# alpenlabs/dv-pari

Measured on AMD Instinct MI355X. Metric: R1CS constraints/sec (prove), higher is better.
Workload: dtype u32; 1 GPU; Proof::prove, synthetic dense R1CS, 2^20 constraints (BASELINE config #4); log2_constraints=20, n_wires=1048576, msm_pairs_per_proof=6291456, witness=resident in HBM, entry=dvp_prove_dev (Proof::prove with the witness resident), proofs_in_flight=1

## Files before the change

dv-pari_amd/csrc/capi.cpp:

```cpp
#include "common.h"

#include <atomic>
#include <map>
#include <mutex>
#include <vector>
#include <cstring>
#include <cstdlib>
#include <climits>

namespace dvp {
thread_local int64_t g_last_error_index = -1;
thread_local hipError_t g_last_hip_error = hipSuccess;

bool g_prof_enabled = false;
static unsigned g_prof_mask = ~0u;
static std::mutex g_prof_mu;
static double g_prof_ms[PROF_NSLOTS] = {0};
static uint64_t g_prof_n[PROF_NSLOTS] = {0};
struct Pending { int slot; hipEvent_t e0, e1; uint64_t key; };
struct Shape { double ms = 0; uint64_t n = 0; };
static std::map<uint64_t, Shape> g_prof_round0;
static std::vector<Pending> g_prof_pending;
static const char* kProfNames[PROF_NSLOTS] = {"msm_affine_round0", "msm_total", "extend_total", "prove_total", "msm_affine_rest", "msm_sort", "msm_tail"};

// ... 6 lines not shown
  if (!e0) return;
  (void)hipEventRecord(e1, st);
  std::lock_guard<std::mutex> g(g_prof_mu);
  g_prof_pending.push_back({slot, e0, e1, key});
  e0 = e1 = nullptr;
}
void prof_collect() {
  std::lock_guard<std::mutex> g(g_prof_mu);
  for (auto& p : g_prof_pending) {
    float ms = 0;
    if (hipEventSynchronize(p.e1) == hipSuccess && hipEventElapsedTime(&ms, p.e0, p.e1) == hipSuccess) {
      g_prof_ms[p.slot] += ms;
      g_prof_n[p.slot] += (p.slot == PROF_MSM_AFFINE_REST && p.key) ? p.key : 1;
      if (p.slot == PROF_MSM_ACCUM_AFFINE && p.key) { Shape& sh = g_prof_round0[p.key]; sh.ms += ms; sh.n += 1; }
    }
    (void)hipEventDestroy(p.e0);
    (void)hipEventDestroy(p.e1);
  }
  g_prof_pending.clear();
}

static std::atomic<uint64_t> g_host_waits[2];
void count_host_wait(int kind) { g_host_waits[kind & 1].fetch_add(1, std::memory_order_relaxed); }

static void tune_from_env(Tune& t) {
  t = Tune();
  auto geti = [](const char* name, long long dflt) { const char* e = getenv(name); return e ? atoll(e) : dflt; };
  t.msm_c = geti("DVP_MSM_C", t.msm_c);
  t.msm_k = geti("DVP_MSM_K", t.msm_k);
  t.msm_fixed_c = geti("DVP_MSM_FIXED_C", t.msm_fixed_c);
  t.fx_hi = geti("DVP_FX_HI", t.fx_hi);
  const char* m = getenv("DVP_MSM_MODE");
  t.msm_proj = (m && !strcmp(m, "proj")) ? 1 : 0;
  t.msm_aff_min = geti("DVP_MSM_AFF_MIN", t.msm_aff_min);
  t.msm_hex_max = geti("DVP_MSM_HEX_MAX", t.msm_hex_max);
  t.msm_round_pipeline = geti("DVP_MSM_ROUND_PIPELINE", t.msm_round_pipeline);
  t.msm_sort_fused = geti("DVP_MSM_SORT_FUSED", t.msm_sort_fused);
  t.msm_bucket_pairs_max = geti("DVP_MSM_BUCKET_PAIRS_MAX", t.msm_bucket_pairs_max);
  t.msm_aff_bmax = geti("DVP_MSM_AFF_BMAX", t.msm_aff_bmax);
  t.msm_aff_bmin = geti("DVP_MSM_AFF_BMIN", t.msm_aff_bmin);
  t.ecfft_radix4 = geti("DVP_ECFFT_RADIX4", t.ecfft_radix4);
  t.ecfft_fold = geti("DVP_ECFFT_FOLD", t.ecfft_fold);
  t.msm_accum_fast = geti("DVP_MSM_ACCUM_FAST", t.msm_accum_fast);
  t.msm_tail_groups = geti("DVP_MSM_TAIL_GROUPS", t.msm_tail_groups);
  t.msm_accum_hex_max = geti("DVP_MSM_ACCUM_HEX_MAX", t.msm_accum_hex_max);
  t.gf_inv_tabs = geti("DVP_GF_INV_TABS", t.gf_inv_tabs);
  t.msm_ws_slots = geti("DVP_MSM_WS_SLOTS", t.msm_ws_slots);
  t.msm_gate_min = geti("DVP_MSM_GATE_MIN", t.msm_gate_min);
  t.msm_aff_tpb = geti("DVP_MSM_AFF_TPB", t.msm_aff_tpb);
  t.cache_replicas = geti("DVP_CACHE_REPLICAS", t.cache_replicas);
  t.msm_quad_max = geti("DVP_MSM_QUAD_MAX", t.msm_quad_max);
  t.msm_accum_quad_max = geti("DVP_MSM_ACCUM_QUAD_MAX", t.msm_accum_quad_max);
  t.msm_fixed_min = geti("DVP_MSM_FIXED_MIN", t.msm_fixed_min);
  t.horner_max_pub = geti("DVP_HORNER_MAX_PUB", t.horner_max_pub);
  t.fr_bi_shape = geti("DVP_FR_BI_SHAPE", t.fr_bi_shape);
  t.msm_aligned_signed = geti("DVP_MSM_ALIGNED_SIGNED", t.msm_aligned_signed);
  t.prove_host_transcript = geti("DVP_PROVE_HOST_TRANSCRIPT", t.prove_host_transcript);
  t.msm_table_refuse = geti("DVP_MSM_TABLE_REFUSE", t.msm_table_refuse);
  if (const char* e = getenv("DVP_TABLE_BUDGET_BYTES")) {
    const unsigned long long v = strtoull(e, nullptr, 10);
    t.table_budget_bytes = v > (unsigned long long)LLONG_MAX ? -1 : (long long)v;
  }
}
static std::mutex g_dev_mu;
static std::vector<int> g_devices;
std::vector<int> mgpu_devices() {
  std::lock_guard<std::mutex> g(g_dev_mu);
  return g_devices;
}
Tune& tune() {
  static Tune t = [] { Tune x; tune_from_env(x); return x; }();
  return t;
}
}

static long long* tune_slot(const char* name) {
  dvp::Tune& t = dvp::tune();
  struct { const char* n; long long* v; } tab[] = {
      {"DVP_MSM_C", &t.msm_c}, {"DVP_MSM_K", &t.msm_k}, {"DVP_MSM_FIXED_C", &t.msm_fixed_c}, {"DVP_FX_HI", &t.fx_hi},
      {"DVP_MSM_PROJ", &t.msm_proj}, {"DVP_MSM_AFF_MIN", &t.msm_aff_min}, {"DVP_MSM_HEX_MAX", &t.msm_hex_max}, {"DVP_MSM_ROUND_PIPELINE", &t.msm_round_pipeline}, {"DVP_MSM_SORT_FUSED", &t.msm_sort_fused}, {"DVP_MSM_BUCKET_PAIRS_MAX", &t.msm_bucket_pairs_max}, {"DVP_MSM_AFF_BMAX", &t.msm_aff_bmax}, {"DVP_MSM_AFF_BMIN", &t.msm_aff_bmin}, {"DVP_ECFFT_RADIX4", &t.ecfft_radix4}, {"DVP_ECFFT_FOLD", &t.ecfft_fold}, {"DVP_MSM_ACCUM_FAST", &t.msm_accum_fast}, {"DVP_MSM_TAIL_GROUPS", &t.msm_tail_groups}, {"DVP_MSM_ACCUM_HEX_MAX", &t.msm_accum_hex_max}, {"DVP_GF_INV_TABS", &t.gf_inv_tabs}, {"DVP_MSM_WS_SLOTS", &t.msm_ws_slots}, {"DVP_MSM_GATE_MIN", &t.msm_gate_min}, {"DVP_MSM_AFF_TPB", &t.msm_aff_tpb}, {"DVP_CACHE_REPLICAS", &t.cache_replicas},
      {"DVP_MSM_QUAD_MAX", &t.msm_quad_max}, {"DVP_MSM_ACCUM_QUAD_MAX", &t.msm_accum_quad_max}, {"DVP_MSM_FIXED_MIN", &t.msm_fixed_min}, {"DVP_HORNER_MAX_PUB", &t.horner_max_pub}, {"DVP_FR_BI_SHAPE", &t.fr_bi_shape},
      {"DVP_MSM_ALIGNED_SIGNED", &t.msm_aligned_signed}, {"DVP_PROVE_HOST_TRANSCRIPT", &t.prove_host_transcript},
      {"DVP_TABLE_BUDGET_BYTES", &t.table_budget_bytes}, {"DVP_MSM_TABLE_REFUSE", &t.msm_table_refuse}};
  for (auto& e : tab)
    if (!strcmp(name, e.n)) return e.v;
  return nullptr;
}
extern "C" int dvp_tune_set(const char* name, long long value) {
  long long* v = name ? tune_slot(name) : nullptr;
  if (!v) return DVP_EINVAL;
  *v = value;
  return DVP_OK;
}
extern "C" int dvp_tune_get(const char* name, long long* value) {
  long long* v = name ? tune_slot(name) : nullptr;
  if (!v || !value) return DVP_EINVAL;
  *value = *v;
  return DVP_OK;
}
extern "C" void dvp_tune_reset(void) { dvp::tune_from_env(dvp::tune()); }

extern "C" void dvp_profile_enable(int on) {
  dvp::g_prof_mask = on == 2 ? (1u << dvp::PROF_MSM_ACCUM_AFFINE) : ~0u;
  dvp::g_prof_enabled = on != 0;
}
extern "C" void dvp_profile_reset(void) {
  dvp::prof_collect();
  std::lock_guard<std::mutex> g(dvp::g_prof_mu);
  for (int i = 0; i < dvp::PROF_NSLOTS; ++i) { dvp::g_prof_ms[i] = 0; dvp::g_prof_n[i] = 0; }
  dvp::g_prof_round0.clear();
  dvp::g_host_waits[0] = 0;
  dvp::g_host_waits[1] = 0;
}
extern "C" int dvp_profile_round0_shapes(uint64_t* pairs, double* total_ms, uint64_t* launches, int cap) {
  if (cap < 0 || (cap > 0 && (!pairs || !total_ms || !launches))) return DVP_EINVAL;
  dvp::prof_collect();
  std::lock_guard<std::mutex> g(dvp::g_prof_mu);
  int k = 0;
  for (auto& e : dvp::g_prof_round0) {
    if (k < cap) { pairs[k] = e.first; total_ms[k] = e.second.ms; launches[k] = e.second.n; }
    ++k;
  }
  return k;
}
extern "C" int dvp_profile_read(const char* name, double* total_ms, uint64_t* launches) {
  if (!name || !total_ms || !launches) return DVP_EINVAL;
  if (!strcmp(name, "host_waits_stream") || !strcmp(name, "host_waits_side")) {
    *total_ms = 0;
    *launches = dvp::g_host_waits[name[11] == 's' && name[12] == 'i' ? 1 : 0].load();
    return DVP_OK;
  }
  dvp::prof_collect();
  std::lock_guard<std::mutex> g(dvp::g_prof_mu);
  for (int i = 0; i < dvp::PROF_NSLOTS; ++i)
    if (!strcmp(name, dvp::kProfNames[i])) { *total_ms = dvp::g_prof_ms[i]; *launches = dvp::g_prof_n[i]; return DVP_OK; }
  return DVP_EINVAL;
}

extern "C" const char* dvp_strerror(int s) {
  switch (s) {
    case DVP_OK: return "ok";
    case DVP_EINVAL: return "invalid argument (size, null pointer or non-canonical field element)";
    case DVP_EDECODE: return "invalid xsk233 point encoding";
    case DVP_EUNSAT: return "R1CS constraint not satisfied by the witness";
    case DVP_EHIP: return "HIP runtime error";
    case DVP_EIO: return "I/O error";
    case DVP_ENOMEM: return "out of memory";
    case DVP_ECHALLENGE: return "Fiat-Shamir challenge lies in the evaluation domain";
    default: return "unknown status";
  }
}

// ... 27 lines not shown
```

dv-pari_amd/csrc/common.h:

```cpp
#pragma once
#include <hip/hip_runtime.h>
#include <stdint.h>
#include <stdio.h>

#include <vector>

#include "../../include/dvpari_internal.h"

namespace dvp {

extern thread_local int64_t g_last_error_index;
extern thread_local hipError_t g_last_hip_error;

inline int hip_fail(hipError_t e, const char* what, const char* file, int line) {
  g_last_hip_error = e;
  fprintf(stderr, "[dvpari] HIP error %d (%s) at %s:%d: %s\n", (int)e, hipGetErrorString(e), file, line, what);
  if (e == hipErrorOutOfMemory) {
    (void)hipGetLastError();
    return DVP_ENOMEM;
  }
  return DVP_EHIP;
}

#define DVP_HIP(call)                                                        \
// ... 40 lines not shown
struct Tune {
  long long msm_c = 0;
  long long msm_k = 0;
  long long msm_fixed_c = 0;
  long long fx_hi = -1;
  long long msm_proj = 0;
  long long msm_aff_min = 1ll << 19;
  long long msm_gate_min = 1;
  long long msm_ws_slots = 2;
  long long cache_replicas = 1;
  long long msm_aff_tpb = 256;
  long long msm_aff_bmin = 8;
  long long msm_aff_bmax = 136;
  long long ecfft_radix4 = 3;
  long long ecfft_fold = 1;
  long long msm_accum_fast = 1;
  long long msm_tail_groups = 1;
  long long msm_accum_hex_max = -1;
  long long gf_inv_tabs = 1;
  long long msm_accum_quad_max = 0;
  long long msm_bucket_pairs_max = 12;
  long long msm_sort_fused = 1;
  long long msm_round_pipeline = 2;
  long long msm_hex_max = -1;
  long long msm_quad_max = 0;
  long long msm_fixed_min = 1ll << 16;
  long long fr_bi_shape = 6;
  long long horner_max_pub = -1;
  long long prove_host_transcript = 0;
  long long table_budget_bytes = -1;
  long long msm_table_refuse = 0;
  long long msm_aligned_signed = 1;
};
Tune& tune();

std::vector<int> mgpu_devices();

inline unsigned cdiv(size_t a, size_t b) { return (unsigned)((a + b - 1) / b); }

enum ProfSlot { PROF_MSM_ACCUM_AFFINE = 0, PROF_MSM_TOTAL, PROF_EXTEND_TOTAL, PROF_PROVE_TOTAL, PROF_MSM_AFFINE_REST, PROF_MSM_SORT, PROF_MSM_TAIL, PROF_NSLOTS };
extern bool g_prof_enabled;
struct ProfScope {
  int slot;
  hipStream_t st;
  hipEvent_t e0 = nullptr, e1 = nullptr;
  uint64_t key = 0;
  ProfScope(int slot_, hipStream_t st_, uint64_t key_ = 0);
  void stop();
};
void prof_collect();
void count_host_wait(int kind);

}
```

dv-pari_amd/csrc/msm.hip:

```cpp
#include <algorithm>
#include <cstdlib>
#include <cstring>
#include <atomic>
#include <chrono>
#include <mutex>
#include <type_traits>
#include <vector>

#include "common.h"
#include "k233.cuh"
#include "tau.cuh"
#include "codec.cuh"

namespace dvp {

constexpr uint32_t FXW_VALID = 0x80000000u, FXW_KEY_MASK = 0xfffffu, FXW_NEG = 0x10000000u, ITEM_NEG = 0x80000000u;
constexpr int FXW_ROW_SHIFT = 20;
__host__ __device__ __forceinline__ uint32_t fxw_key(uint32_t d) { return d & FXW_KEY_MASK; }
__host__ __device__ __forceinline__ uint32_t fxw_row(uint32_t d) { return (d >> FXW_ROW_SHIFT) & 0xffu; }

template <class DIGIT>
__global__ void __launch_bounds__(256)
k_recode(const uint32_t* __restrict__ scalars, const uint8_t* __restrict__ inf, uint32_t n, int c, int W, int n_narrow,
         DIGIT* __restrict__ digits, unsigned long long* __restrict__ err) {
// ... 1030 lines not shown
  const uint32_t base = blockIdx.x * SCAN_BLK + threadIdx.x * SCAN_EPT;
  for (int r = 1; r <= R; ++r) {
    uint32_t* o = rp + (size_t)(2 * (r - 1) + 1) * ((size_t)m + 1);
    const uint32_t add = bs[(size_t)(r - 1) * gridDim.x + blockIdx.x];
    if (r == 1 && off0) {
#pragma unroll
      for (int k = 0; k < SCAN_EPT; ++k)
        if (base + k < m) {
          const uint32_t v = o[base + k] + add, c = cnt0[base + k];
          o[base + k] = v;
          off0[base + k] = 2u * v;
          if (c & 1u) items[2u * v + c] = AFF_NONE;
        }
      continue;
    }
#pragma unroll
    for (int k = 0; k < SCAN_EPT; ++k)
      if (base + k < m) o[base + k] += add;
  }
}
struct DescPlan {
  unsigned long long at[40];
};
template <int LPK>
__global__ void __launch_bounds__(1024)
k_round_desc_all(const uint32_t* __restrict__ rp, uint32_t nkeys, int R, DescPlan plan, uint32_t* __restrict__ desc) {
  const uint32_t gid = blockIdx.x * blockDim.x + threadIdx.x;
  const uint32_t key = gid / LPK, lane = gid % LPK;
  if (key >= nkeys) return;
  const size_t stride = (size_t)nkeys + 1;
  for (int r0 = 1; r0 < R; r0 += 8) {
    uint32_t cr[8], o[8], oo[8];
#pragma unroll
    for (int q = 0; q < 8; ++q) {
      const int r = r0 + q;
      if (r < R) {
        const uint32_t* c = rp + (size_t)(2 * (r - 1)) * stride;
        cr[q] = c[key];
        o[q] = c[stride + key];
        oo[q] = c[3 * stride + key];
      } else {
        cr[q] = 0; o[q] = 0; oo[q] = 0;
      }
    }
#pragma unroll
    for (int q = 0; q < 8; ++q) {
      const int r = r0 + q;
      if (r >= R) break;
      const uint32_t nout = (cr[q] + 1) >> 1;
      uint32_t* d = desc + plan.at[r];
      for (uint32_t j = lane; j < nout; j += LPK) d[oo[q] + j] = (o[q] + 2 * j) | ((2 * j + 1 < cr[q]) ? DESC_PAIR : 0u);
    }
  }
}

template <int LPK>
__global__ void __launch_bounds__(256)
k_round_desc(const uint32_t* __restrict__ cnt, const uint32_t* __restrict__ off, const uint32_t* __restrict__ ooff ,
             uint32_t nkeys, uint32_t* __restrict__ desc) {
  const uint32_t gid = blockIdx.x * blockDim.x + threadIdx.x;
  const uint32_t key = gid / LPK, lane = gid % LPK;
  if (key >= nkeys) return;
  const uint32_t c = cnt[key], o = off[key], oo = ooff[key], nout = (c + 1) >> 1;
  for (uint32_t j = lane; j < nout; j += LPK) desc[oo + j] = (o + 2 * j) | ((2 * j + 1 < c) ? DESC_PAIR : 0u);
}

#ifndef AFF_PRIO
#define AFF_PRIO 1
#endif
#ifndef AFF_XY
#define AFF_XY 1
#endif
__device__ __forceinline__ void aff_set_prio(uint32_t v) {
  switch (v % 3u) {
    case 0: __builtin_amdgcn_s_setprio(0); break;
    case 1: __builtin_amdgcn_s_setprio(1); break;
    default: __builtin_amdgcn_s_setprio(2); break;
  }
}
constexpr uint32_t AFF_BMAX = 136;
__device__ __forceinline__ uint32_t aff_slots_per_thread(uint32_t total, uint32_t cap, uint32_t bmax_bmin) {
  const uint32_t bmax = bmax_bmin & 0xffu, bmin = (bmax_bmin >> 8) & 0xffu;
  const uint32_t units = (total + cap - 1) / cap;
  const uint32_t R = (units + bmax - 1) / bmax;
  const uint32_t B = R ? (units + R - 1) / R : 1;
  return B < bmin ? bmin : B;
}
struct WaveTrace {
  unsigned long long* buf;
  uint32_t cap, tag;
};
template <bool FIRST, bool TRACE = false>
__global__ void __launch_bounds__(EC_TPB) __attribute__((amdgpu_waves_per_eu(3, 3)))
k_affine_round(const Aff* __restrict__ pts, const uint2* __restrict__ desc, const uint32_t* __restrict__ total_ptr ,
               uint32_t cap, uint32_t bmax, GfSqrTables T, Gf* __restrict__ prefix, Aff* __restrict__ out, uint32_t sign_mask, WaveTrace wt) {
  extern __shared__ char lds_raw[];
  unsigned long long tr_t0 = 0, tr_c0 = 0, tr_t1 = 0, tr_t2 = 0;
  if (TRACE) { tr_t0 = wall_clock64(); tr_c0 = clock64(); }
  GfLdsK L = gf_ldsk_init(lds_raw);
#if AFF_PRIO
  const uint32_t wslot = __builtin_amdgcn_s_getreg(((4 - 1) << 11) | 4);
#endif
  const uint32_t sm = FIRST ? sign_mask : 0u;
  auto ldx = [&](uint32_t v) -> Gf { return pts[v & ~sm].x; };
  auto ldy = [&](uint32_t v, const Gf& x) -> Gf {
    Gf y = pts[v & ~sm].y;
    if (v & sm) y = gf_add(y, x);
    return y;
  };
  const uint32_t total = *total_ptr;
  const int B = (int)aff_slots_per_thread(total, cap, bmax);
  const uint32_t nthr = (total + B - 1) / B;
  const uint32_t tid = blockIdx.x * blockDim.x + threadIdx.x;
  if (tid >= nthr) return;
  const uint2 none = make_uint2(AFF_NONE, AFF_NONE);
  auto ld_desc = [&](int k) -> uint2 {
    const uint32_t sk = (uint32_t)k * nthr + tid;
    const bool ok = k >= 0 && k < B && sk < total;
    if (FIRST) {
      uint2 v = none;
      if (ok) v = desc[sk];
      return v;
    }
    const uint32_t d = ((const uint32_t*)desc)[ok ? sk : 0u], a = d & ~DESC_PAIR;
    return make_uint2(ok ? a : AFF_NONE, (ok && (d & DESC_PAIR)) ? a + 1 : AFF_NONE);
  };
  const Gf one = gf_one();
  Gf run = one;
  {
    uint2 d0 = ld_desc(0), d1 = ld_desc(1);
    Gf xa = gf_zero(), xb = gf_zero();
    if (d0.y != AFF_NONE) { xa = ldx(d0.x); xb = ldx(d0.y); }
#pragma unroll 1
    for (int k = 0; k < B; ++k) {
#if AFF_PRIO
      aff_set_prio(wslot + (uint32_t)k);
#endif
      const uint2 d2 = ld_desc(k + 2);
      Gf nxa = gf_zero(), nxb = gf_zero();
      if (d1.y != AFF_NONE) { nxa = ldx(d1.x); nxb = ldx(d1.y); }
      Gf den = one;
      if (d0.y != AFF_NONE && !gf_is_zero(xa) && !gf_is_zero(xb)) {
        Gf dd = gf_add(xa, xb);
        if (!gf_is_zero(dd)) den = dd;
        else if (gf_eq(ldy(d0.x, xa), ldy(d0.y, xb))) den = xa;
      }
      prefix[(size_t)k * nthr + tid] = run;
      run = gf_mul(run, den, L);
      d0 = d1; d1 = d2; xa = nxa; xb = nxb;
    }
  }
  if (TRACE) tr_t1 = wall_clock64();
  Gf inv = gf_inv_fast(run, T, L);
  if (TRACE) tr_t2 = wall_clock64();
  {
    uint2 e0 = ld_desc(B - 1), e1 = ld_desc(B - 2);
    Gf px = gf_zero(), qx = gf_zero(), pre = one;
    if (e0.x != AFF_NONE) px = ldx(e0.x);
    if (e0.y != AFF_NONE) { qx = ldx(e0.y); pre = prefix[(size_t)(B - 1) * nthr + tid]; }
#if AFF_XY
    Gf py = gf_zero(), qy = gf_zero();
    if (e0.x != AFF_NONE) py = ldy(e0.x, px);
    if (e0.y != AFF_NONE) qy = ldy(e0.y, qx);
#endif
#pragma unroll 1
    for (int k = B - 1; k >= 0; --k) {
#if AFF_PRIO
      aff_set_prio(wslot + (uint32_t)k);
#endif
      const uint2 e2 = ld_desc(k - 2);
#if AFF_XY
      Gf npx = gf_zero(), nqx = gf_zero(), npy = gf_zero(), nqy = gf_zero(), npre = one;
      if (e1.x != AFF_NONE) { npx = ldx(e1.x); npy = ldy(e1.x, npx); }
      if (e1.y != AFF_NONE) { nqx = ldx(e1.y); nqy = ldy(e1.y, nqx); npre = prefix[(size_t)(k - 1) * nthr + tid]; }
#else
      Gf py = gf_zero(), qy = gf_zero();
      if (e0.x != AFF_NONE) py = ldy(e0.x, px);
      if (e0.y != AFF_NONE) qy = ldy(e0.y, qx);
      Gf npx = gf_zero(), nqx = gf_zero(), npre = one;
      if (e1.x != AFF_NONE) npx = ldx(e1.x);
      if (e1.y != AFF_NONE) { nqx = ldx(e1.y); npre = prefix[(size_t)(k - 1) * nthr + tid]; }
#endif
      if (e0.x != AFF_NONE) {
        const uint32_t sidx = (uint32_t)k * nthr + tid;
        Gf ox = px, oy = py;
        if (e0.y != AFF_NONE) {
          if (gf_is_zero(px)) { ox = qx; oy = qy; }
          else if (!gf_is_zero(qx)) {
            Gf dd = gf_add(px, qx);
            const bool same_x = gf_is_zero(dd);
            const bool dbl = same_x && gf_eq(py, qy);
            if (same_x && !dbl) {
              ox = gf_zero(); oy = gf_zero();
            } else {
              Gf den = dbl ? px : dd;
              Gf dinv, inv_next;
              gf_mul2(pre, den, inv, L, dinv, inv_next);
              inv = inv_next;
              Gf num = dbl ? py : gf_add(py, qy);
              Gf lam = gf_mul(num, dinv, L);
              if (dbl) lam = gf_add(lam, px);
              ox = gf_add(gf_add(gf_sqr(lam), lam), dd);
              oy = gf_add(gf_add(gf_mul(gf_add(px, ox), lam, L), ox), py);
            }
          }
        }
        out[sidx].x = ox; out[sidx].y = oy;
      }
      e0 = e1; e1 = e2; px = npx; qx = nqx; pre = npre;
#if AFF_XY
      py = npy; qy = nqy;
#endif
    }
  }
#if AFF_PRIO
  __builtin_amdgcn_s_setprio(0);
#endif
  if (TRACE) {
    const unsigned long long t3 = wall_clock64(), c3 = clock64();
    if ((threadIdx.x & 63u) == 0) {
      const unsigned long long i = atomicAdd(wt.buf, 1ull);
      if (i < wt.cap) {
        unsigned long long* r = wt.buf + 8 + 8 * i;
        r[0] = tr_t0; r[1] = tr_t1; r[2] = tr_t2; r[3] = t3;
        r[4] = tr_c0; r[5] = c3;
        r[6] = (unsigned long long)__builtin_amdgcn_s_getreg((31 << 11) | 4) | ((unsigned long long)__builtin_amdgcn_s_getreg((31 << 11) | 20) << 32);
        r[7] = (unsigned long long)blockIdx.x | ((unsigned long long)wt.tag << 32) | ((unsigned long long)(uint32_t)B << 48);
      }
    }
  }
}

__global__ void __launch_bounds__(256)
k_bucket_gather_aff(const Aff* __restrict__ in, const uint32_t* __restrict__ cnt, const uint32_t* __restrict__ off,
// ... 497 lines not shown
    static std::mutex attr_mu;
    static bool attr_done[MSM_MAX_DEVICES] = {false};
    std::lock_guard<std::mutex> ga(attr_mu);
    if (!attr_done[cur_dev]) {
      hipError_t attr_err = hipFuncSetAttribute((const void*)k_scatter_local, hipFuncAttributeMaxDynamicSharedMemorySize, 131072);
      if (attr_err == hipSuccess)
        attr_err = hipFuncSetAttribute((const void*)k_hist_local, hipFuncAttributeMaxDynamicSharedMemorySize, 65536);
      if (attr_err == hipSuccess)
        attr_err = hipFuncSetAttribute((const void*)k_scatter_local2, hipFuncAttributeMaxDynamicSharedMemorySize, 131072);
      if (attr_err == hipSuccess)
        attr_err = hipFuncSetAttribute((const void*)k_hist_local2, hipFuncAttributeMaxDynamicSharedMemorySize, 65536);
      if (attr_err == hipSuccess)
        attr_err = hipFuncSetAttribute((const void*)k_part_scatter_staged, hipFuncAttributeMaxDynamicSharedMemorySize, FX_STAGE1_LDS);
      if (attr_err == hipSuccess)
        attr_err = hipFuncSetAttribute((const void*)k_part_scatter_signed<true>, hipFuncAttributeMaxDynamicSharedMemorySize, FX_STAGE1_LDS);
      if (attr_err == hipSuccess)
        attr_err = hipFuncSetAttribute((const void*)k_scatter_local2_staged, hipFuncAttributeMaxDynamicSharedMemorySize, FX_STAGE2_LDS);
      const void* ec[] = {(const void*)k_accum_affine<true, false>, (const void*)k_accum_affine<false, false>, (const void*)k_accum_affine<true, true>,
                          (const void*)k_accum_affine<false, true>, (const void*)k_accum_proj<1>, (const void*)k_accum_proj<4>, (const void*)k_accum_proj<16>,
                          (const void*)k_accum_affine_fast<true, false>, (const void*)k_accum_affine_fast<false, false>, (const void*)k_accum_affine_fast<true, true>,
                          (const void*)k_accum_affine_fast<false, true>, (const void*)k_accum_affine_rest<true>, (const void*)k_accum_affine_rest<false>,
                          (const void*)k_tail_groups, (const void*)k_merge<1, false>, (const void*)k_merge<4, false>, (const void*)k_merge<16, false>, (const void*)k_merge<1, true>, (const void*)k_merge<4, true>, (const void*)k_merge<16, true>,
                          (const void*)k_affine_round<true, false>, (const void*)k_affine_round<false, false>, (const void*)k_affine_round<true, true>,
                          (const void*)k_affine_round<false, true>, (const void*)k_sum_points, (const void*)k_tail<false>, (const void*)k_tail<true>,
                          (const void*)k_bucket_pairs, (const void*)k_bucket_rest};
      for (const void* f : ec)
        if (attr_err == hipSuccess) attr_err = hipFuncSetAttribute(f, hipFuncAttributeMaxDynamicSharedMemorySize, EC_LDS_Q);
      DVP_HIP(attr_err);
      attr_done[cur_dev] = true;
    }
  }
  MsmPlan p = msm_plan(n, fx);
  const FxBits fb = fx ? fx->bits() : FxBits{0, 0};
  const uint32_t FX_NP = fb.np();
  std::unique_lock<std::mutex> g;
  int ws_slot = 0;
  const int ws_slots = tune().msm_ws_slots >= 1 && tune().msm_ws_slots <= MSM_WS_SLOTS ? (int)tune().msm_ws_slots : 1;
  for (int pass = 0; pass < 2 && !g.owns_lock(); ++pass)
    for (int sl = 0; sl < ws_slots && !g.owns_lock(); ++sl) {
      g = std::unique_lock<std::mutex>(g_ws_dev[cur_dev][sl].mu, std::try_to_lock);
      if (g.owns_lock() && pass == 0 && g_ws_dev[cur_dev][sl].busy_for(st)) g.unlock();
      if (g.owns_lock()) ws_slot = sl;
    }
  if (!g.owns_lock()) g = std::unique_lock<std::mutex>(g_ws_dev[cur_dev][0].mu);
  MsmWorkspace& g_ws = g_ws_dev[cur_dev][ws_slot];
  if (g_ws.busy_valid) {
    if (g_ws.busy_stream != st) DVP_HIP(hipStreamWaitEvent(st, g_ws.ev_busy, 0));
// ... 19 lines not shown
  size_t o_ntask = carve(((size_t)p.nkeys + 1) * 4);
  size_t o_toff = carve(((size_t)p.nkeys + 1) * 4);
  size_t o_cnt2 = carve(((size_t)p.nkeys + 1) * 4);
  size_t o_off2 = carve(((size_t)p.nkeys + 1) * 4);
  size_t o_bsum = carve(((size_t)p.nkeys / SCAN_BLK + 8) * 4);
  size_t o_items = carve((p.e_max + (size_t)p.nkeys + 2) * 4);
  const size_t sort_cells = fx ? ((size_t)(fx_nblk + FX_NP + 1) << fb.lo) : ((size_t)p.W * cdiv(n, SORT_CHUNK) << p.c);
  size_t o_hist16 = carve(sort_cells * 2);
  size_t o_choff = carve(sort_cells * 4);
  size_t o_bufA = carve(p.t1_max * sizeof(Ld));
  size_t o_bufB = carve(p.t2_max * sizeof(Ld));
  const Tune tn = tune();
  const bool affine_mode = !tn.msm_proj;
  const size_t affA_n = p.e_max / 2 + p.nkeys + 1, affB_n = p.e_max / 4 + p.nkeys + 1;
  size_t o_affA = carve(affine_mode ? affA_n * sizeof(Aff) : 16);
  size_t o_affB = carve(affine_mode ? affB_n * sizeof(Aff) : 16);
  size_t o_prefix = carve(affine_mode ? (affA_n + 256) * sizeof(Gf) : 16);
  const size_t aff_min = (size_t)(tn.msm_aff_min > 0 ? tn.msm_aff_min : 1);
  const size_t e_est = (size_t)n * (size_t)((fx && fx->signed_digits) ? p.W : (234 + p.c - 1) / p.c);
  int ra_plan = 0;
  while (affine_mode && ra_plan < 40 && (e_est >> (ra_plan + 1)) >= aff_min) ++ra_plan;
  const bool pipelined = affine_mode && tn.msm_round_pipeline != 0 && ra_plan >= 2 && e_est >= 4 * (size_t)p.nkeys;
  const bool side_stream = pipelined && tn.msm_round_pipeline == 1;
  std::vector<size_t> desc_at((size_t)ra_plan + 1, 0);
  size_t desc_n = affA_n + 64;
  if (pipelined) {
    size_t cap_r = p.e_max + p.nkeys, at = 0;
    for (int r = 0; r < ra_plan; ++r) {
      const size_t out_max = cap_r / 2 + p.nkeys + 1;
      if (r >= 1) { desc_at[r] = at; at += out_max + 64; }
      cap_r = out_max;
    }
    if (at > desc_n) desc_n = at;
  }
  size_t o_gdesc = carve(affine_mode ? desc_n * sizeof(uint32_t) : 16);
  size_t o_rp = carve(pipelined ? (size_t)ra_plan * 2 * ((size_t)p.nkeys + 1) * 4 : 16);
  size_t o_bsum2 = carve(((size_t)((ra_plan > 0 ? ra_plan : 1) + 1) * ((size_t)p.nkeys / SCAN_BLK + 1) + 8) * 4);
  size_t o_bkt = carve((size_t)p.nkeys * sizeof(Ld));
  const size_t rest_cap = (size_t)p.nkeys + 2 + p.e_max / (size_t)(p.K > 0 ? p.K : 1);
  size_t o_rest = carve(rest_cap * 4);
  const uint32_t tail_groups = ((uint32_t)(p.W * p.c) + 15u) / 16u;
  size_t o_tail = carve(((size_t)2 * p.W * p.c + 1 + 2 * (size_t)tail_groups) * sizeof(Ld));
  DVP_TRY(g_ws.ensure(o, g_ws_need[cur_dev]));
  char* base = (char*)g_ws.p;
  auto* err = (unsigned long long*)(base + o_err);
  auto* digits = (uint16_t*)(base + o_digits);
  auto* digits32 = (uint32_t*)(base + o_digits32);
  auto* plo = (uint16_t*)(base + o_plo);
  auto* pid = (uint32_t*)(base + o_pid);
  auto* phist = (uint32_t*)(base + o_phist);
  auto* pbase = (uint32_t*)(base + o_pbase);
  auto* ctot = (uint32_t*)(base + o_ctot);
  auto* pstart = (uint32_t*)(base + o_pstart);
// ... 41 lines not shown
    DVP_HIP(hipStreamWaitEvent(g_ws.aux, g_ws.ev, 0));
    DVP_HIP(hipMemcpyAsync(g_ws.pinned, d_max, 4, hipMemcpyDeviceToHost, g_ws.aux));
    return DVP_OK;
  };
  const bool sort_done_by_mscan = pipelined && !side_stream;
  auto prepare_rounds = [&]() -> int {
    if (!pipelined) return DVP_OK;
    hipStream_t bk = st;
    if (side_stream) {
      DVP_TRY(g_ws.ensure_side(1));
      DVP_HIP(hipEventRecord(g_ws.ev_pre, st));
      DVP_HIP(hipStreamWaitEvent(g_ws.side, g_ws.ev_pre, 0));
      bk = g_ws.side;
    }
    const uint32_t nb = cdiv(nk, SCAN_BLK);
    uint32_t* off0 = side_stream ? nullptr : off;
    hipLaunchKernelGGL(k_mscan_local, dim3(nb), dim3(SCAN_TPB), 0, bk, cnt, nk, ra_plan, rp, bsum2);
    hipLaunchKernelGGL(k_mscan_bsums, dim3(ra_plan), dim3(SCAN_TPB), 0, bk, bsum2, nb, nk, rp, off0, off0 ? d_max : (uint32_t*)nullptr);
    if (off0) DVP_TRY(read_max());
    hipLaunchKernelGGL(k_mscan_add, dim3(nb), dim3(SCAN_TPB), 0, bk, rp, bsum2, nk, ra_plan, (const uint32_t*)cnt, off0, items);
    DescPlan plan;
    for (int q = 0; q < 40; ++q) plan.at[q] = q < ra_plan ? desc_at[q] : 0;
    const size_t per_key = (e_est >> 2) / nk;
    if (per_key >= 48)
      hipLaunchKernelGGL((k_round_desc_all<64>), dim3(cdiv((size_t)nk * 64, 1024)), dim3(1024), 0, bk, rp, nk, ra_plan, plan, gdesc);
    else if (per_key >= 8)
      hipLaunchKernelGGL((k_round_desc_all<16>), dim3(cdiv((size_t)nk * 16, 1024)), dim3(1024), 0, bk, rp, nk, ra_plan, plan, gdesc);
    else
      hipLaunchKernelGGL((k_round_desc_all<4>), dim3(cdiv((size_t)nk * 4, 1024)), dim3(1024), 0, bk, rp, nk, ra_plan, plan, gdesc);
    if (side_stream) DVP_HIP(hipEventRecord(g_ws.ev_side[0], g_ws.side));
    DVP_HIP(hipGetLastError());
    prepared = ra_plan;
    return DVP_OK;
  };
  ProfScope ps_total(PROF_MSM_TOTAL, st);
  ProfScope ps_sort(PROF_MSM_SORT, st);
  if (!g_ws.ctrl_clean) {
    DVP_HIP(hipMemsetAsync(err, 0xff, 8, st));
    DVP_HIP(hipMemsetAsync(err + 1, 0, 8, st));
  }
  g_ws.ctrl_clean = false;
  if (fused1)
    ;
  else if (fx && fx->signed_digits)
    hipLaunchKernelGGL(k_recode_signed, dim3(cdiv(n, 256)), dim3(256), 0, st, (const uint32_t*)d_scalars, (const uint8_t*)d_inf, (uint32_t)n,
                       p.c, p.W, p.n_narrow, digits32, err);
  else if (fx)
    hipLaunchKernelGGL((k_recode<uint32_t>), dim3(cdiv(n, 256)), dim3(256), 0, st, (const uint32_t*)d_scalars, (const uint8_t*)d_inf,
                       (uint32_t)n, p.c, p.W, p.n_narrow, digits32, err);
  else
    hipLaunchKernelGGL((k_recode<uint16_t>), dim3(cdiv(n, 256)), dim3(256), 0, st, (const uint32_t*)d_scalars, (const uint8_t*)d_inf,
                       (uint32_t)n, p.c, p.W, p.n_narrow, digits, err);
// ... 59 lines not shown
  const uint32_t aff_lds = (aff_tpb / 64) * GF_LDSK_BYTES_PER_WAVE;
  DVP_HIP(hipOccupancyMaxActiveBlocksPerMultiprocessor(&blk_per_cu, (const void*)k_affine_round<false, false>, (int)aff_tpb, aff_lds));
  if (blk_per_cu < 1) blk_per_cu = 1;
  const uint32_t aff_cap = (uint32_t)n_cu * (uint32_t)blk_per_cu * aff_tpb;
  const uint32_t aff_bmax_only = tn.msm_aff_bmax >= 1 && tn.msm_aff_bmax <= 255 ? (uint32_t)tn.msm_aff_bmax : AFF_BMAX;
  const uint32_t aff_bmin = tn.msm_aff_bmin >= 1 && (uint32_t)tn.msm_aff_bmin <= aff_bmax_only ? (uint32_t)tn.msm_aff_bmin : 1u;
  const uint32_t aff_bmax = aff_bmax_only | (aff_bmin << 8);
  unsigned long long* wt_buf = nullptr;
  uint32_t wt_cap = 0;
  wave_trace_snapshot(&wt_buf, &wt_cap);
  const bool wt_on = wt_buf != nullptr;
  auto launch_round = [&](int r, const uint32_t* d_total, const uint2* dsc) -> int {
    size_t out_max = cap / 2 + nk + 1;
    Aff* outp = (r & 1) ? affB : affA;
    const uint32_t r_max = cdiv(cdiv(out_max, aff_cap), aff_bmax_only);
    const uint32_t grid = r_max * (aff_cap / aff_tpb) + 1;
    {
      ProfScope ps0(r == 0 ? PROF_MSM_ACCUM_AFFINE : -1, st, (uint64_t)n);
      WaveTrace wt{wt_buf, wt_cap, g_wave_trace_tag.fetch_add(wt_on ? 1u : 0u)};
      if (r == 0 && wt.buf)
        hipLaunchKernelGGL((k_affine_round<true, true>), dim3(grid), dim3(aff_tpb), aff_lds, st, pts_in, dsc, d_total, aff_cap, aff_bmax, Tsq, prefix, outp, sign_mask, wt);
      else if (r == 0)
        hipLaunchKernelGGL((k_affine_round<true, false>), dim3(grid), dim3(aff_tpb), aff_lds, st, pts_in, dsc, d_total, aff_cap, aff_bmax, Tsq, prefix, outp, sign_mask, wt);
      else if (wt.buf)
        hipLaunchKernelGGL((k_affine_round<false, true>), dim3(grid), dim3(aff_tpb), aff_lds, st, pts_in, dsc, d_total, aff_cap, aff_bmax, Tsq, prefix, outp, 0u, wt);
      else
        hipLaunchKernelGGL((k_affine_round<false, false>), dim3(grid), dim3(aff_tpb), aff_lds, st, pts_in, dsc, d_total, aff_cap, aff_bmax, Tsq, prefix, outp, 0u, wt);
      ps0.stop();
    }
    pts_in = outp;
    cap = out_max;
    return DVP_OK;
  };
  auto run_round = [&](int r) -> int {
    if (pipelined) {
      if (r == 0 && side_stream) DVP_HIP(hipStreamWaitEvent(st, g_ws.ev_side[0], 0));
      DVP_TRY(launch_round(r, ro(r + 1) + nk, r == 0 ? (const uint2*)items : (const uint2*)(const void*)(gdesc + desc_at[r])));
      return DVP_OK;
    }
    const int nxt = (cur + 1) % 3;
    if (r == 0) {
      if (!(r0_offsets_ready && cur == 0))
        hipLaunchKernelGGL(k_round0_offsets, dim3(cdiv(nk + 1, 256)), dim3(256), 0, st, pc[cur], po[cur], nk, pc[nxt], po[nxt]);
    } else
      DVP_TRY(bookkeep(r, pc[cur], po[cur], pc[nxt], po[nxt], gdesc, st, bsum));
    DVP_TRY(launch_round(r, po[nxt] + nk, r == 0 ? (const uint2*)items : (const uint2*)(const void*)gdesc));
    cur = nxt;
    return DVP_OK;
  };
  int launched = 0;
  std::unique_lock<std::mutex> heavy;
// ... 525 lines not shown
```

Measured before the change: 56.07 million constraints/s.

## Fold numerator into batched-inversion prefix and add optional dense round descriptors

The affine round kernel now multiplies the pair numerator (ya+yb) into the forward prefix product, so the backward pass yields lambda directly from a single paired multiply instead of an inverse followed by a separate multiply. This removes one field multiply and the qy load from the backward pass, at the cost of loading both y coordinates in the forward pass. It also adds an opt-in dense descriptor layout for later rounds that carries explicit output slots and skips wave iterations with no pairs, plus counters for later-round launches. The dense layout doubles descriptor storage and is off by default.

```diff
diff --git a/dv-pari_amd/csrc/capi.cpp b/dv-pari_amd/csrc/capi.cpp
--- a/dv-pari_amd/csrc/capi.cpp
+++ b/dv-pari_amd/csrc/capi.cpp
@@ -52,6 +52,8 @@
 
 static std::atomic<uint64_t> g_host_waits[2];
 void count_host_wait(int kind) { g_host_waits[kind & 1].fetch_add(1, std::memory_order_relaxed); }
+static std::atomic<uint64_t> g_later_rounds[2];
+void count_later_round(bool dense) { g_later_rounds[dense ? 1 : 0].fetch_add(1, std::memory_order_relaxed); }
 
 static void tune_from_env(Tune& t) {
   t = Tune();
@@ -65,6 +67,7 @@
   t.msm_aff_min = geti("DVP_MSM_AFF_MIN", t.msm_aff_min);
   t.msm_hex_max = geti("DVP_MSM_HEX_MAX", t.msm_hex_max);
   t.msm_round_pipeline = geti("DVP_MSM_ROUND_PIPELINE", t.msm_round_pipeline);
+  t.msm_round_dense = geti("DVP_MSM_ROUND_DENSE", t.msm_round_dense);
   t.msm_sort_fused = geti("DVP_MSM_SORT_FUSED", t.msm_sort_fused);
   t.msm_bucket_pairs_max = geti("DVP_MSM_BUCKET_PAIRS_MAX", t.msm_bucket_pairs_max);
   t.msm_aff_bmax = geti("DVP_MSM_AFF_BMAX", t.msm_aff_bmax);
@@ -108,7 +111,7 @@
   dvp::Tune& t = dvp::tune();
   struct { const char* n; long long* v; } tab[] = {
       {"DVP_MSM_C", &t.msm_c}, {"DVP_MSM_K", &t.msm_k}, {"DVP_MSM_FIXED_C", &t.msm_fixed_c}, {"DVP_FX_HI", &t.fx_hi},
-      {"DVP_MSM_PROJ", &t.msm_proj}, {"DVP_MSM_AFF_MIN", &t.msm_aff_min}, {"DVP_MSM_HEX_MAX", &t.msm_hex_max}, {"DVP_MSM_ROUND_PIPELINE", &t.msm_round_pipeline}, {"DVP_MSM_SORT_FUSED", &t.msm_sort_fused}, {"DVP_MSM_BUCKET_PAIRS_MAX", &t.msm_bucket_pairs_max}, {"DVP_MSM_AFF_BMAX", &t.msm_aff_bmax}, {"DVP_MSM_AFF_BMIN", &t.msm_aff_bmin}, {"DVP_ECFFT_RADIX4", &t.ecfft_radix4}, {"DVP_ECFFT_FOLD", &t.ecfft_fold}, {"DVP_MSM_ACCUM_FAST", &t.msm_accum_fast}, {"DVP_MSM_TAIL_GROUPS", &t.msm_tail_groups}, {"DVP_MSM_ACCUM_HEX_MAX", &t.msm_accum_hex_max}, {"DVP_GF_INV_TABS", &t.gf_inv_tabs}, {"DVP_MSM_WS_SLOTS", &t.msm_ws_slots}, {"DVP_MSM_GATE_MIN", &t.msm_gate_min}, {"DVP_MSM_AFF_TPB", &t.msm_aff_tpb}, {"DVP_CACHE_REPLICAS", &t.cache_replicas},
+      {"DVP_MSM_PROJ", &t.msm_proj}, {"DVP_MSM_AFF_MIN", &t.msm_aff_min}, {"DVP_MSM_HEX_MAX", &t.msm_hex_max}, {"DVP_MSM_ROUND_PIPELINE", &t.msm_round_pipeline}, {"DVP_MSM_ROUND_DENSE", &t.msm_round_dense}, {"DVP_MSM_SORT_FUSED", &t.msm_sort_fused}, {"DVP_MSM_BUCKET_PAIRS_MAX", &t.msm_bucket_pairs_max}, {"DVP_MSM_AFF_BMAX", &t.msm_aff_bmax}, {"DVP_MSM_AFF_BMIN", &t.msm_aff_bmin}, {"DVP_ECFFT_RADIX4", &t.ecfft_radix4}, {"DVP_ECFFT_FOLD", &t.ecfft_fold}, {"DVP_MSM_ACCUM_FAST", &t.msm_accum_fast}, {"DVP_MSM_TAIL_GROUPS", &t.msm_tail_groups}, {"DVP_MSM_ACCUM_HEX_MAX", &t.msm_accum_hex_max}, {"DVP_GF_INV_TABS", &t.gf_inv_tabs}, {"DVP_MSM_WS_SLOTS", &t.msm_ws_slots}, {"DVP_MSM_GATE_MIN", &t.msm_gate_min}, {"DVP_MSM_AFF_TPB", &t.msm_aff_tpb}, {"DVP_CACHE_REPLICAS", &t.cache_replicas},
       {"DVP_MSM_QUAD_MAX", &t.msm_quad_max}, {"DVP_MSM_ACCUM_QUAD_MAX", &t.msm_accum_quad_max}, {"DVP_MSM_FIXED_MIN", &t.msm_fixed_min}, {"DVP_HORNER_MAX_PUB", &t.horner_max_pub}, {"DVP_FR_BI_SHAPE", &t.fr_bi_shape},
       {"DVP_MSM_ALIGNED_SIGNED", &t.msm_aligned_signed}, {"DVP_PROVE_HOST_TRANSCRIPT", &t.prove_host_transcript},
       {"DVP_TABLE_BUDGET_BYTES", &t.table_budget_bytes}, {"DVP_MSM_TABLE_REFUSE", &t.msm_table_refuse}};
@@ -141,6 +144,8 @@
   dvp::g_prof_round0.clear();
   dvp::g_host_waits[0] = 0;
   dvp::g_host_waits[1] = 0;
+  dvp::g_later_rounds[0] = 0;
+  dvp::g_later_rounds[1] = 0;
 }
 extern "C" int dvp_profile_round0_shapes(uint64_t* pairs, double* total_ms, uint64_t* launches, int cap) {
   if (cap < 0 || (cap > 0 && (!pairs || !total_ms || !launches))) return DVP_EINVAL;
@@ -158,6 +163,11 @@
   if (!strcmp(name, "host_waits_stream") || !strcmp(name, "host_waits_side")) {
     *total_ms = 0;
     *launches = dvp::g_host_waits[name[11] == 's' && name[12] == 'i' ? 1 : 0].load();
+    return DVP_OK;
+  }
+  if (!strcmp(name, "later_rounds_word") || !strcmp(name, "later_rounds_dense")) {
+    *total_ms = 0;
+    *launches = dvp::g_later_rounds[name[13] == 'd' ? 1 : 0].load();
     return DVP_OK;
   }
   dvp::prof_collect();
diff --git a/dv-pari_amd/csrc/common.h b/dv-pari_amd/csrc/common.h
--- a/dv-pari_amd/csrc/common.h
+++ b/dv-pari_amd/csrc/common.h
@@ -86,6 +86,7 @@
   long long msm_bucket_pairs_max = 12;
   long long msm_sort_fused = 1;
   long long msm_round_pipeline = 2;
+  long long msm_round_dense = 0;
   long long msm_hex_max = -1;
   long long msm_quad_max = 0;
   long long msm_fixed_min = 1ll << 16;
@@ -114,5 +115,6 @@
 };
 void prof_collect();
 void count_host_wait(int kind);
+void count_later_round(bool dense);
 
 }
diff --git a/dv-pari_amd/csrc/msm.hip b/dv-pari_amd/csrc/msm.hip
--- a/dv-pari_amd/csrc/msm.hip
+++ b/dv-pari_amd/csrc/msm.hip
@@ -1076,7 +1076,7 @@
 struct DescPlan {
   unsigned long long at[40];
 };
-template <int LPK>
+template <int LPK, bool DENSE>
 __global__ void __launch_bounds__(1024)
 k_round_desc_all(const uint32_t* __restrict__ rp, uint32_t nkeys, int R, DescPlan plan, uint32_t* __restrict__ desc) {
   const uint32_t gid = blockIdx.x * blockDim.x + threadIdx.x;
@@ -1084,7 +1084,7 @@
   if (key >= nkeys) return;
   const size_t stride = (size_t)nkeys + 1;
   for (int r0 = 1; r0 < R; r0 += 8) {
-    uint32_t cr[8], o[8], oo[8];
+    uint32_t cr[8], o[8], oo[8], A[8];
 #pragma unroll
     for (int q = 0; q < 8; ++q) {
       const int r = r0 + q;
@@ -1093,8 +1093,9 @@
         cr[q] = c[key];
         o[q] = c[stride + key];
         oo[q] = c[3 * stride + key];
+        A[q] = DENSE ? c[stride + nkeys] - c[3 * stride + nkeys] : 0u;
       } else {
-        cr[q] = 0; o[q] = 0; oo[q] = 0;
+        cr[q] = 0; o[q] = 0; oo[q] = 0; A[q] = 0;
       }
     }
 #pragma unroll
@@ -1103,6 +1104,13 @@
       if (r >= R) break;
       const uint32_t nout = (cr[q] + 1) >> 1;
       uint32_t* d = desc + plan.at[r];
+      if (DENSE) {
+        const uint32_t npair = cr[q] >> 1, a = o[q] - oo[q];
+        uint2* d2 = (uint2*)d;
+        for (uint32_t j = lane; j < npair; j += LPK) d2[a + j] = make_uint2((o[q] + 2 * j) | DESC_PAIR, oo[q] + j);
+        if ((cr[q] & 1u) && lane == npair % LPK) d2[A[q] + (2 * oo[q] - o[q])] = make_uint2(o[q] + cr[q] - 1, oo[q] + npair);
+        continue;
+      }
       for (uint32_t j = lane; j < nout; j += LPK) d[oo[q] + j] = (o[q] + 2 * j) | ((2 * j + 1 < cr[q]) ? DESC_PAIR : 0u);
     }
   }
@@ -1125,6 +1133,9 @@
 #ifndef AFF_XY
 #define AFF_XY 1
 #endif
+#ifndef AFF_NUM1
+#define AFF_NUM1 1
+#endif
 __device__ __forceinline__ void aff_set_prio(uint32_t v) {
   switch (v % 3u) {
     case 0: __builtin_amdgcn_s_setprio(0); break;
@@ -1144,7 +1155,10 @@
   unsigned long long* buf;
   uint32_t cap, tag;
 };
-template <bool FIRST, bool TRACE = false>
+struct AffSlot {
+  uint32_t a, b, o;
+};
+template <bool FIRST, bool TRACE = false, bool DENSE = false>
 __global__ void __launch_bounds__(EC_TPB) __attribute__((amdgpu_waves_per_eu(3, 3)))
 k_affine_round(const Aff* __restrict__ pts, const uint2* __restrict__ desc, const uint32_t* __restrict__ total_ptr ,
                uint32_t cap, uint32_t bmax, GfSqrTables T, Gf* __restrict__ prefix, Aff* __restrict__ out, uint32_t sign_mask, WaveTrace wt) {
@@ -1168,91 +1182,141 @@
   const uint32_t tid = blockIdx.x * blockDim.x + threadIdx.x;
   if (tid >= nthr) return;
   const uint2 none = make_uint2(AFF_NONE, AFF_NONE);
-  auto ld_desc = [&](int k) -> uint2 {
+  auto ld_desc = [&](int k) -> AffSlot {
     const uint32_t sk = (uint32_t)k * nthr + tid;
     const bool ok = k >= 0 && k < B && sk < total;
     if (FIRST) {
       uint2 v = none;
       if (ok) v = desc[sk];
-      return v;
-    }
-    const uint32_t d = ((const uint32_t*)desc)[ok ? sk : 0u], a = d & ~DESC_PAIR;
-    return make_uint2(ok ? a : AFF_NONE, (ok && (d & DESC_PAIR)) ? a + 1 : AFF_NONE);
+      return AffSlot{v.x, v.y, 0u};
+    }
+    const uint2 d = DENSE ? desc[ok ? sk : 0u] : make_uint2(((const uint32_t*)desc)[ok ? sk : 0u], 0u);
+    const uint32_t a = d.x & ~DESC_PAIR;
+    return AffSlot{ok ? a : AFF_NONE, (ok && (d.x & DESC_PAIR)) ? a + 1 : AFF_NONE, d.y};
   };
   const Gf one = gf_one();
   Gf run = one;
   {
-    uint2 d0 = ld_desc(0), d1 = ld_desc(1);
+    AffSlot d0 = ld_desc(0), d1 = ld_desc(1);
     Gf xa = gf_zero(), xb = gf_zero();
-    if (d0.y != AFF_NONE) { xa = ldx(d0.x); xb = ldx(d0.y); }
+    if (d0.b != AFF_NONE) { xa = ldx(d0.a); xb = ldx(d0.b); }
+#if AFF_NUM1
+    Gf ya = gf_zero(), yb = gf_zero();
+    if (d0.b != AFF_NONE) { ya = ldy(d0.a, xa); yb = ldy(d0.b, xb); }
+#endif
 #pragma unroll 1
     for (int k = 0; k < B; ++k) {
 #if AFF_PRIO
       aff_set_prio(wslot + (uint32_t)k);
 #endif
-      const uint2 d2 = ld_desc(k + 2);
+      const AffSlot d2 = ld_desc(k + 2);
       Gf nxa = gf_zero(), nxb = gf_zero();
-      if (d1.y != AFF_NONE) { nxa = ldx(d1.x); nxb = ldx(d1.y); }
-      Gf den = one;
-      if (d0.y != AFF_NONE && !gf_is_zero(xa) && !gf_is_zero(xb)) {
-        Gf dd = gf_add(xa, xb);
-        if (!gf_is_zero(dd)) den = dd;
-        else if (gf_eq(ldy(d0.x, xa), ldy(d0.y, xb))) den = xa;
+      if (d1.b != AFF_NONE) { nxa = ldx(d1.a); nxb = ldx(d1.b); }
+#if AFF_NUM1
+      Gf nya = gf_zero(), nyb = gf_zero();
+      if (d1.b != AFF_NONE) { nya = ldy(d1.a, nxa); nyb = ldy(d1.b, nxb); }
+#endif
+      const bool pair = d0.b != AFF_NONE;
+      if (!DENSE || __any(pair)) {
+        Gf den = one;
+#if AFF_NUM1
+        Gf num = gf_zero();
+        if (pair && !gf_is_zero(xa) && !gf_is_zero(xb)) {
+          const Gf dd = gf_add(xa, xb), ys = gf_add(ya, yb);
+          if (!gf_is_zero(dd)) { den = dd; num = ys; }
+          else if (gf_is_zero(ys)) { den = xa; num = ya; }
+        }
+        Gf np, nrun;
+        gf_mul2(num, den, run, L, np, nrun);
+        if (pair) prefix[(size_t)k * nthr + tid] = np;
+        run = nrun;
+#else
+        if (pair && !gf_is_zero(xa) && !gf_is_zero(xb)) {
+          Gf dd = gf_add(xa, xb);
+          if (!gf_is_zero(dd)) den = dd;
+          else if (gf_eq(ldy(d0.a, xa), ldy(d0.b, xb))) den = xa;
+        }
+        if (pair) prefix[(size_t)k * nthr + tid] = run;
+        run = gf_mul(run, den, L);
+#endif
       }
-      prefix[(size_t)k * nthr + tid] = run;
-      run = gf_mul(run, den, L);
       d0 = d1; d1 = d2; xa = nxa; xb = nxb;
+#if AFF_NUM1
+      ya = nya; yb = nyb;
+#endif
     }
   }
   if (TRACE) tr_t1 = wall_clock64();
   Gf inv = gf_inv_fast(run, T, L);
   if (TRACE) tr_t2 = wall_clock64();
   {
-    uint2 e0 = ld_desc(B - 1), e1 = ld_desc(B - 2);
+    AffSlot e0 = ld_desc(B - 1), e1 = ld_desc(B - 2);
     Gf px = gf_zero(), qx = gf_zero(), pre = one;
-    if (e0.x != AFF_NONE) px = ldx(e0.x);
-    if (e0.y != AFF_NONE) { qx = ldx(e0.y); pre = prefix[(size_t)(B - 1) * nthr + tid]; }
+    if (e0.a != AFF_NONE) px = ldx(e0.a);
+    if (e0.b != AFF_NONE) { qx = ldx(e0.b); pre = prefix[(size_t)(B - 1) * nthr + tid]; }
 #if AFF_XY
-    Gf py = gf_zero(), qy = gf_zero();
-    if (e0.x != AFF_NONE) py = ldy(e0.x, px);
-    if (e0.y != AFF_NONE) qy = ldy(e0.y, qx);
+    Gf py = gf_zero();
+    if (e0.a != AFF_NONE) py = ldy(e0.a, px);
+#if !AFF_NUM1
+    Gf qy = gf_zero();
+    if (e0.b != AFF_NONE) qy = ldy(e0.b, qx);
+#endif
 #endif
 #pragma unroll 1
     for (int k = B - 1; k >= 0; --k) {
 #if AFF_PRIO
       aff_set_prio(wslot + (uint32_t)k);
 #endif
-      const uint2 e2 = ld_desc(k - 2);
+      const AffSlot e2 = ld_desc(k - 2);
 #if AFF_XY
-      Gf npx = gf_zero(), nqx = gf_zero(), npy = gf_zero(), nqy = gf_zero(), npre = one;
-      if (e1.x != AFF_NONE) { npx = ldx(e1.x); npy = ldy(e1.x, npx); }
-      if (e1.y != AFF_NONE) { nqx = ldx(e1.y); nqy = ldy(e1.y, nqx); npre = prefix[(size_t)(k - 1) * nthr + tid]; }
+      Gf npx = gf_zero(), nqx = gf_zero(), npy = gf_zero(), npre = one;
+      if (e1.a != AFF_NONE) { npx = ldx(e1.a); npy = ldy(e1.a, npx); }
+#if AFF_NUM1
+      if (e1.b != AFF_NONE) { nqx = ldx(e1.b); npre = prefix[(size_t)(k - 1) * nthr + tid]; }
 #else
-      Gf py = gf_zero(), qy = gf_zero();
-      if (e0.x != AFF_NONE) py = ldy(e0.x, px);
-      if (e0.y != AFF_NONE) qy = ldy(e0.y, qx);
+      Gf nqy = gf_zero();
+      if (e1.b != AFF_NONE) { nqx = ldx(e1.b); nqy = ldy(e1.b, nqx); npre = prefix[(size_t)(k - 1) * nthr + tid]; }
+#endif
+#else
+      Gf py = gf_zero();
+      if (e0.a != AFF_NONE) py = ldy(e0.a, px);
+#if !AFF_NUM1
+      Gf qy = gf_zero();
+      if (e0.b != AFF_NONE) qy = ldy(e0.b, qx);
+#endif
       Gf npx = gf_zero(), nqx = gf_zero(), npre = one;
-      if (e1.x != AFF_NONE) npx = ldx(e1.x);
-      if (e1.y != AFF_NONE) { nqx = ldx(e1.y); npre = prefix[(size_t)(k - 1) * nthr + tid]; }
+      if (e1.a != AFF_NONE) npx = ldx(e1.a);
+      if (e1.b != AFF_NONE) { nqx = ldx(e1.b); npre = prefix[(size_t)(k - 1) * nthr + tid]; }
 #endif
-      if (e0.x != AFF_NONE) {
-        const uint32_t sidx = (uint32_t)k * nthr + tid;
+#if AFF_NUM1
+      auto q_y = [&]() -> Gf { return ldy(e0.b, qx); };
+#else
+      auto q_y = [&]() -> Gf { return qy; };
+#endif
+      if (e0.a != AFF_NONE) {
+        const uint32_t sidx = DENSE ? e0.o : (uint32_t)k * nthr + tid;
         Gf ox = px, oy = py;
-        if (e0.y != AFF_NONE) {
-          if (gf_is_zero(px)) { ox = qx; oy = qy; }
+        if (e0.b != AFF_NONE) {
+          if (gf_is_zero(px)) { ox = qx; oy = q_y(); }
           else if (!gf_is_zero(qx)) {
             Gf dd = gf_add(px, qx);
             const bool same_x = gf_is_zero(dd);
-            const bool dbl = same_x && gf_eq(py, qy);
+            const bool dbl = same_x && gf_eq(py, q_y());
             if (same_x && !dbl) {
               ox = gf_zero(); oy = gf_zero();
             } else {
               Gf den = dbl ? px : dd;
+#if AFF_NUM1
+              Gf lam, inv_next;
+              gf_mul2(pre, den, inv, L, lam, inv_next);
+              inv = inv_next;
+#else
               Gf dinv, inv_next;
               gf_mul2(pre, den, inv, L, dinv, inv_next);
               inv = inv_next;
               Gf num = dbl ? py : gf_add(py, qy);
               Gf lam = gf_mul(num, dinv, L);
+#endif
               if (dbl) lam = gf_add(lam, px);
               ox = gf_add(gf_add(gf_sqr(lam), lam), dd);
               oy = gf_add(gf_add(gf_mul(gf_add(px, ox), lam, L), ox), py);
@@ -1263,7 +1327,10 @@
       }
       e0 = e1; e1 = e2; px = npx; qx = nqx; pre = npre;
 #if AFF_XY
-      py = npy; qy = nqy;
+      py = npy;
+#if !AFF_NUM1
+      qy = nqy;
+#endif
 #endif
     }
   }
@@ -1807,7 +1874,8 @@
                           (const void*)k_accum_affine_fast<false, true>, (const void*)k_accum_affine_rest<true>, (const void*)k_accum_affine_rest<false>,
                           (const void*)k_tail_groups, (const void*)k_merge<1, false>, (const void*)k_merge<4, false>, (const void*)k_merge<16, false>, (const void*)k_merge<1, true>, (const void*)k_merge<4, true>, (const void*)k_merge<16, true>,
                           (const void*)k_affine_round<true, false>, (const void*)k_affine_round<false, false>, (const void*)k_affine_round<true, true>,
-                          (const void*)k_affine_round<false, true>, (const void*)k_sum_points, (const void*)k_tail<false>, (const void*)k_tail<true>,
+                          (const void*)k_affine_round<false, true>, (const void*)k_affine_round<false, false, true>, (const void*)k_affine_round<false, true, true>,
+                          (const void*)k_sum_points, (const void*)k_tail<false>, (const void*)k_tail<true>,
                           (const void*)k_bucket_pairs, (const void*)k_bucket_rest};
       for (const void* f : ec)
         if (attr_err == hipSuccess) attr_err = hipFuncSetAttribute(f, hipFuncAttributeMaxDynamicSharedMemorySize, EC_LDS_Q);
@@ -1873,13 +1941,14 @@
   while (affine_mode && ra_plan < 40 && (e_est >> (ra_plan + 1)) >= aff_min) ++ra_plan;
   const bool pipelined = affine_mode && tn.msm_round_pipeline != 0 && ra_plan >= 2 && e_est >= 4 * (size_t)p.nkeys;
   const bool side_stream = pipelined && tn.msm_round_pipeline == 1;
+  const bool dense = pipelined && tn.msm_round_dense != 0;
   std::vector<size_t> desc_at((size_t)ra_plan + 1, 0);
   size_t desc_n = affA_n + 64;
   if (pipelined) {
     size_t cap_r = p.e_max + p.nkeys, at = 0;
     for (int r = 0; r < ra_plan; ++r) {
       const size_t out_max = cap_r / 2 + p.nkeys + 1;
-      if (r >= 1) { desc_at[r] = at; at += out_max + 64; }
+      if (r >= 1) { desc_at[r] = at; at += (dense ? 2 : 1) * (out_max + 64); }
       cap_r = out_max;
     }
     if (at > desc_n) desc_n = at;
@@ -1967,12 +2036,11 @@
     DescPlan plan;
     for (int q = 0; q < 40; ++q) plan.at[q] = q < ra_plan ? desc_at[q] : 0;
     const size_t per_key = (e_est >> 2) / nk;
-    if (per_key >= 48)
-      hipLaunchKernelGGL((k_round_desc_all<64>), dim3(cdiv((size_t)nk * 64, 1024)), dim3(1024), 0, bk, rp, nk, ra_plan, plan, gdesc);
-    else if (per_key >= 8)
-      hipLaunchKernelGGL((k_round_desc_all<16>), dim3(cdiv((size_t)nk * 16, 1024)), dim3(1024), 0, bk, rp, nk, ra_plan, plan, gdesc);
-    else
-      hipLaunchKernelGGL((k_round_desc_all<4>), dim3(cdiv((size_t)nk * 4, 1024)), dim3(1024), 0, bk, rp, nk, ra_plan, plan, gdesc);
+    const int lpk = per_key >= 48 ? 64 : per_key >= 8 ? 16 : 4;
+    auto desc_all = lpk == 64 ? (dense ? k_round_desc_all<64, true> : k_round_desc_all<64, false>)
+                  : lpk == 16 ? (dense ? k_round_desc_all<16, true> : k_round_desc_all<16, false>)
+                              : (dense ? k_round_desc_all<4, true> : k_round_desc_all<4, false>);
+    hipLaunchKernelGGL(desc_all, dim3(cdiv((size_t)nk * lpk, 1024)), dim3(1024), 0, bk, rp, nk, ra_plan, plan, gdesc);
     if (side_stream) DVP_HIP(hipEventRecord(g_ws.ev_side[0], g_ws.side));
     DVP_HIP(hipGetLastError());
     prepared = ra_plan;
@@ -2078,11 +2146,16 @@
         hipLaunchKernelGGL((k_affine_round<true, true>), dim3(grid), dim3(aff_tpb), aff_lds, st, pts_in, dsc, d_total, aff_cap, aff_bmax, Tsq, prefix, outp, sign_mask, wt);
       else if (r == 0)
         hipLaunchKernelGGL((k_affine_round<true, false>), dim3(grid), dim3(aff_tpb), aff_lds, st, pts_in, dsc, d_total, aff_cap, aff_bmax, Tsq, prefix, outp, sign_mask, wt);
+      else if (dense && wt.buf)
+        hipLaunchKernelGGL((k_affine_round<false, true, true>), dim3(grid), dim3(aff_tpb), aff_lds, st, pts_in, dsc, d_total, aff_cap, aff_bmax, Tsq, prefix, outp, 0u, wt);
+      else if (dense)
+        hipLaunchKernelGGL((k_affine_round<false, false, true>), dim3(grid), dim3(aff_tpb), aff_lds, st, pts_in, dsc, d_total, aff_cap, aff_bmax, Tsq, prefix, outp, 0u, wt);
       else if (wt.buf)
         hipLaunchKernelGGL((k_affine_round<false, true>), dim3(grid), dim3(aff_tpb), aff_lds, st, pts_in, dsc, d_total, aff_cap, aff_bmax, Tsq, prefix, outp, 0u, wt);
       else
         hipLaunchKernelGGL((k_affine_round<false, false>), dim3(grid), dim3(aff_tpb), aff_lds, st, pts_in, dsc, d_total, aff_cap, aff_bmax, Tsq, prefix, outp, 0u, wt);
       ps0.stop();
+      if (r > 0) count_later_round(dense);
     }
     pts_in = outp;
     cap = out_max;
```

Result: faster. 58.13 million constraints/s, median of 6 (+3.7%).
